# EasyVision-Ton/VMG

Hardware: AMD Instinct MI355X
Metric: LR-frames/s (train: forward+loss+backward+AdamW), VMG-REDS-few_levels 4x SR (higher is better)
Workload: dtype bf16; 1 GPU; VMG-REDS-few_levels train step, per-GPU batch 4x7x3x64x64 -> 4x SR (BASELINE configs[1]); global_batch=4, frames_per_clip=7, parallelism=dp1, launch=eager, recompute_chains=False, fp8_chains=False

## Files before the change

include/vmg_hip.h:

```cpp
#ifndef VMG_HIP_H
#define VMG_HIP_H

#include <stdint.h>

#ifdef __cplusplus
extern "C" {
#endif

#define VMG_F32 0
#define VMG_BF16 1

#define VMG_ACT_NONE 0
#define VMG_ACT_RELU 1
#define VMG_ACT_LRELU 2
#define VMG_ACT_GELU 3

#define VMG_CONV_GENERAL 0
#define VMG_CONV_KSPLIT 2
#define VMG_CONV_WS 3
#define VMG_CONV_LINEAR_WRES 4
#define VMG_CONV_WSTAT 6

const char* vmg_last_error(void);
int vmg_version(void);
// ... 36 lines not shown
  int deep;
} vmg_conv_desc;

int vmg_conv_fwd(const vmg_conv_desc* d, void* stream);
typedef struct vmg_chain_desc {
  int dtype, N, H, W, C, nblk, nsrc;
  const void* src[4];
  int64_t src_ps[4];
  int src_ch[4];
  const void* packed0;
  const float* bias0;
  float slope0;
  int cout_tiles0, deep0;
  const void* const* packed1;
  const float* const* bias1;
  const void* const* packed2;
  const float* const* bias2;
  float r_scaling;
  int cout_tiles, deep;
  void* const* y;
  void* const* t;
  void* const* g_y;
  void* const* g_t;
} vmg_chain_desc;
int vmg_resblock_chain_fwd(const vmg_chain_desc* d, void* stream);
int vmg_resblock_chain_bwd(const vmg_chain_desc* d, void* stream);

void* vmg_replay_build(void* hip_graph, int* n_ops, int* n_kernels);
int vmg_replay_kernel_info(void* replay, int idx, void** func, unsigned* grid_x, unsigned* block_x, void** first_arg);
int vmg_replay_run(void* replay, int first, int last, void* stream);
void vmg_replay_destroy(void* replay);

int vmg_pack_entry_bytes(void);
int vmg_pack_entry(void* entry, int kind, int dtype, const float* w, int O, int I, int ks, int o0, int on, int nsrc, const int* src_off,
                   const int* src_ch, int transpose_flip, int cout_tiles, void* packed, int blk0);
int vmg_pack_run(const void* plan_dev, int n, int total_blocks, void* stream);

int vmg_conv_debug_stamps(void* buf);

int vmg_conv_wgrad(int dtype, int ks, int N, int H, int W, const void* x, int64_t x_ps, int Cin, const void* dy,
                   int64_t dy_ps, int Cout, float* dW, int I_total, int o0, int i0, float* db, float scale,
                   void* stream);
int vmg_conv_wgrad_batched(int dtype, int ks, int npairs, const void* const* x, const void* const* dy, int N, int H, int W,
                           int64_t x_ps, int Cin, int64_t dy_ps, int Cout, float* dW, int I_total, int o0, int i0, float* db,
                           float scale, void* stream);

int64_t vmg_conv_wgrad_ws_bytes(void);
int vmg_conv_wgrad_batched_ws(int dtype, int ks, int npairs, const void* const* x, const void* const* dy, int N, int H, int W,
                              int64_t x_ps, int Cin, int64_t dy_ps, int Cout, float* dW, int I_total, int o0, int i0, float* db,
                              float scale, void* ws, int64_t ws_bytes, void* stream);
int vmg_conv_wgrad3_multi(int nprob, int npairs, const void* const* x, const void* const* dy, int N, int H, int W, int64_t x_ps, int Cin,
                          int64_t dy_ps, int Cout, float* const* dW, int I_total, int o0, int i0, float* const* db, const float* scales, void* ws,
                          int64_t ws_bytes, void* stream);
int vmg_conv_wgrad3_variant(int variant);
int vmg_linear_wgrad2_multi(int nprob, int npairs, const void* const* x, const void* const* dy, int64_t M, int64_t x_ps, int Cin, int64_t dy_ps,
                            int Cout, float* const* dW, int I_total, int o0, int i0, float* const* db, const float* scales, void* ws,
                            int64_t ws_bytes, void* stream);
#define VMG_WGRAD_V1 1
#define VMG_WGRAD_3 2
#define VMG_WGRAD_3B 3
#define VMG_WGRAD_L2 4
#define VMG_WGRAD_7 5
int vmg_conv_wgrad_last_kernel(void);
#define VMG_WGRAD_ENTRY_PLAIN 0
#define VMG_WGRAD_ENTRY_WS 1
#define VMG_WGRAD_ENTRY_MULTI 2
#define VMG_WGRAD_ALIGN_X16 1
#define VMG_WGRAD_ALIGN_DY16 2
#define VMG_WGRAD_ALIGN_DY2 4
#define VMG_WGRAD_PLAN_INTS 7
int vmg_conv_wgrad_plan(int entry, int dtype, int ks, int nprob, int npairs, int N, int H, int W, int64_t x_ps, int Cin, int64_t dy_ps, int Cout,
                        int I_total, int o0, int i0, int align, int64_t ws_bytes, int* plan);

int vmg_act_bwd(int dtype, const void* dy, const void* ref, void* out, int64_t n, int act, float slope, float alpha,
                void* stream);
int vmg_pixel_shuffle(int dtype, const void* in, void* out, int N, int H, int W, int c, int to_depth, void* stream);
int vmg_sum_n(int dtype, const void* const* srcs, int nsrc, void* out, int64_t n, void* stream);
int vmg_cast_clear(int dtype, float* acc, const void* add, void* out, int64_t n, void* stream);
int vmg_pair_steps(int dtype, int mode, void* const* steps, void* a, void* b, int n, int t, int64_t frame_elems, void* stream);
int vmg_frame_gather(int dtype, const void* src, void* dst, const int* idx, int64_t frame_elems, int n_src_frames, int n_dst_frames, int nsrc,
                     void* stream);
int vmg_pixel_unshuffle_actgrad(int dtype, const void* dy, const void* ref, void* out, int N, int H, int W, int c, int act, float slope,
                                float alpha, void* stream);
int vmg_layernorm_fwd(int dtype, const void* x, const float* w, const float* b, void* y, float* mean, float* rstd, int64_t M,
                      int C, float eps, void* stream);
int64_t vmg_layernorm_bwd_ws_bytes(void);
int vmg_layernorm_bwd(int dtype, int ndy, const void* const* dy, const void* x, const float* mean, const float* rstd, const float* w,
                      const void* add, void* dx, float* dw, float* db, int64_t M, int C, void* ws, void* stream);

int vmg_space_depth_ln_fwd(int dtype, int mode, const void* x, const float* w, const float* b, void* y, float* mean, float* rstd, int N, int H,
                           int W, int cseg, float eps, void* stream);
int vmg_space_depth_ln_bwd(int dtype, int mode, const void* dy, const void* x, const float* mean, const float* rstd, const float* w, void* dx,
                           float* dw, float* db, int N, int H, int W, int cseg, void* ws, void* stream);

int64_t vmg_group_reduce_ws_bytes(void);
int vmg_group_reduce(int dtype, const void* a, const void* b, const void* c3, float* out, int G, int64_t R, int C, int mode, float scale,
                     float* ws, int64_t ws_bytes, void* stream);
int vmg_group_reduce3(int dtype, const void* a, const void* b0, const void* b1, const void* b2, float* out, int G, int64_t R, int C, float scale,
                      float* ws, int64_t ws_bytes, void* stream);
int vmg_tab_elementwise(int dtype, int op, const void* p0, const void* p1, const void* p2, const float* coef, const float* add, float s,
                        void* o0, void* o1, void* o2, int64_t rows, int64_t R, int C, void* stream);

int vmg_warp_bilinear_fwd(int dtype, const void* x, const float* flow, void* out, int N, int H, int W, int C, void* stream);
int vmg_warp_bilinear_bwd(int dtype, const void* x, const float* flow, const void* dy, void* dx_acc, float* dflow, int N, int H,
                          int W, int C, void* stream);
int vmg_warp_nearest_planes(const float* loc, const float* flow, float* out, int N, int K2, int H, int W, void* stream);
// ... 157 lines not shown
```

vmg_amd/csrc/conv_wgrad.hip:

```cpp
#include <stdlib.h>
#include <algorithm>
#include <type_traits>

#include "common.h"

namespace {

constexpr int WG_MAX_PAIRS = 16;
int g_last_kernel = 0;
constexpr int last_kernel_id(int kind, int a = 0, int b = 0, int c = 0) { return kind << 24 | a << 16 | b << 8 | c; }
__device__ __attribute__((aligned(256))) unsigned int g_zero_buf[64];

__device__ __forceinline__ void glds16_hidden(const char* gsrc, char* lds_dst) {
  unsigned keep;
  const unsigned ldst = __builtin_amdgcn_readfirstlane((unsigned)(uintptr_t)LDS_PTR(lds_dst));
  asm volatile("s_mov_b32 %0, m0\n\ts_mov_b32 m0, %2\n\ts_nop 0\n\tglobal_load_lds_dwordx4 %1, off\n\ts_mov_b32 m0, %0"
               : "=&s"(keep) : "v"(gsrc), "s"(ldst) : "memory");
}

struct SlabBlock { int x, y, z; };
__device__ __forceinline__ SlabBlock xcd_slab_block(int gx, int gy, int S) {
  const int T = gx * gy * S, L = blockIdx.x;
  const int xcd = L & 7, j = L >> 3, rem = T & 7;
  const int w = xcd * (T >> 3) + (xcd < rem ? xcd : rem) + j;
// ... 518 lines not shown
#pragma unroll
    for (int jj = 0; jj < 7; ++jj) {
#ifdef VMG_DIAG
      if (!(a.dbg & 2))
#endif
      {
#pragma unroll
        for (int c = 0; c < 5; ++c) acc[c][jj] = __builtin_amdgcn_mfma_f32_16x16x32_bf16(af[c], bfg[jj], acc[c][jj], 0, 0, 0);
      }
#ifdef VMG_DIAG
      if (!(a.dbg & 4))
#endif
      bfg[jj] = tr_read(src + b_off[jj], W2_XC * 2);
    }
#ifdef VMG_DIAG
    if (!(a.dbg & 4))
#endif
    {
#pragma unroll
      for (int c = 0; c < 5; ++c) af[c] = tr_read(src + a_off + c * 32, W2_DYC * 2);
    }
    if (SYNC && h == 1) {
#ifdef VMG_DIAG
      if (!(a.dbg & 1))
#endif
      {
        if (j + 5 < nun) issue(S5);
        if (j + 6 < nun) issue(SU);
      }
    }
    return true;
  };
  for (int base = 0; base < nun; base += 6) {
    if (!unit(base + 0, std::integral_constant<int, 0>{})) break;
    if (!unit(base + 1, std::integral_constant<int, 1>{})) break;
    if (!unit(base + 2, std::integral_constant<int, 2>{})) break;
    if (!unit(base + 3, std::integral_constant<int, 3>{})) break;
    if (!unit(base + 4, std::integral_constant<int, 4>{})) break;
    if (!unit(base + 5, std::integral_constant<int, 5>{})) break;
  }
  asm volatile("s_waitcnt lgkmcnt(0)" ::: "memory");
  float* sl = a.slab + ((((long long)zz * a.gy + blk.y) * a.gx + blk.x) * W3_WAVES + wave) * (W3_TILES * 256);
#pragma unroll
  for (int c = 0; c < 5; ++c)
#pragma unroll
    for (int j = 0; j < 7; ++j) *reinterpret_cast<f32x4*>(sl + ((c * 7 + j) * 64 + lane) * 4) = acc[c][j];
  if (a.has_bias && q == 0 && blk.y == 0) {
    f32x4 pack = f32x4{0.f, 0.f, 0.f, 0.f};
    if (li < 5) pack = li == 0 ? accb[0] : (li == 1 ? accb[1] : (li == 2 ? accb[2] : (li == 3 ? accb[3] : accb[4])));
    *reinterpret_cast<f32x4*>(sl + (35 * 64 + lane) * 4) = pack;
  }
}

__global__ __launch_bounds__(W3_THREADS) void conv_wgrad3b_kernel(const Wgrad2K a) {
  extern __shared__ __attribute__((aligned(16))) char smem[];
  const int tid = threadIdx.x, lane = tid & 63;
  const int wave = __builtin_amdgcn_readfirstlane(tid >> 6);
  const int h = wave >> 2, q = wave & 3;
  SlabBlock blk = xcd_slab_block(a.gx, a.gy, a.S * a.nprob);
  const int prob = blk.z / a.S;
  const int zz = blk.z;
  blk.z -= prob * a.S;
  const char* const* xs = a.x + prob * WG_MAX_PAIRS;
  const char* const* dys = a.dy + prob * WG_MAX_PAIRS;
  const int ob = blk.x * W2_DYC, ib = blk.y * W2_XC;
  const long long u_lo = a.U * blk.z / a.S, u_hi = a.U * (blk.z + 1) / a.S;
  const char* zsrc = reinterpret_cast<const char*>(g_zero_buf);

  f32x4 acc[5][7];
#pragma unroll
  for (int c = 0; c < 5; ++c)
#pragma unroll
    for (int j = 0; j < 7; ++j) acc[c][j] = f32x4{0.f, 0.f, 0.f, 0.f};
  const bf16 one = (bf16)1.0f;
  const bf16x8 ones = {one, one, one, one, one, one, one, one};
  const bool bias_col = q == 3;

  unsigned voff[W3_SLOTS], flg[W3_SLOTS];
  const int nun = (int)(u_hi - u_lo);
  int ipair = (int)(u_lo / a.Upair), iseg, iy, in_;
  {
    const long long uu = u_lo - (long long)ipair * a.Upair;
    iseg = (int)(uu % a.SEG);
    const long long r = uu / a.SEG;
    iy = (int)(r % a.H);
    in_ = (int)(r / a.H);
  }
  const int wlast = a.W - (a.SEG - 1) * 32;
#pragma unroll
  for (int sl = 0; sl < W3_SLOTS; ++sl) {
    const int L = (sl * W3_WAVES + wave) * 64 + lane;
    if (L < W3_DYV) {
      const int pp = L / 18, v = L - pp * 18;
      voff[sl] = (unsigned)((pp * a.dy_ps + ob + v * 8) * 2);
      flg[sl] = 32u | (pp >= wlast ? 8u : 0u) | ((ob + v * 8 + 8 <= a.Cout) ? 0u : 16u);
    } else if (L < W3_VECS) {
      const int vec = L - W3_DYV, pp = vec / 6, v = vec - pp * 6;
      const int rr = pp / W2_XW, col = pp - rr * W2_XW;
      voff[sl] = (unsigned)(((long long)(rr * a.W + col) * a.x_ps + ib + v * 8) * 2);
      flg[sl] = 32u | (rr == 0 ? 1u : 0u) | (rr == 2 ? 2u : 0u) | (col == 0 ? 4u : 0u) | (col - 1 >= wlast ? 8u : 0u) | ((ib + v * 8 + 8 <= a.Cin) ? 0u : 16u);
    } else {
      voff[sl] = 0u;
      flg[sl] = 48u;
    }
  }
  const long long halo_x = (long long)(a.W + 1) * a.x_ps * 2;
  w3_u32x4 rs_dy = w3_rsrc(dys[ipair]), rs_x = w3_rsrc(xs[ipair] - halo_x);
// ... 74 lines not shown
    const char* src = smem + ((j + 1 < nun) ? SN : SU) * W3_BUF;
#ifdef VMG_DIAG
    const bool nocopy = a.dbg & 1;
#else
    constexpr bool nocopy = false;
#endif
    if (SYNC && h == 0) {
      issue(S5, j + 5 < nun && !nocopy);
      issue(SU, j + 6 < nun && !nocopy);
    }
#pragma unroll
    for (int jj = 0; jj < 7; ++jj) {
#ifdef VMG_DIAG
      if (!(a.dbg & 2))
#endif
      {
#pragma unroll
        for (int c = 0; c < 5; ++c) acc[c][jj] = __builtin_amdgcn_mfma_f32_16x16x32_bf16(af[c], bfg[jj], acc[c][jj], 0, 0, 0);
      }
#ifdef VMG_DIAG
      if (!(a.dbg & 4))
#endif
      if (jj < 6 || !bias_col) bfg[jj] = tr_read(src + b_off[jj], W2_XC * 2);
    }
#ifdef VMG_DIAG
    if (!(a.dbg & 4))
#endif
    {
#pragma unroll
      for (int c = 0; c < 5; ++c) af[c] = tr_read(src + a_off + c * 32, W2_DYC * 2);
    }
    if (SYNC && h == 1) {
      issue(S5, j + 5 < nun && !nocopy);
      issue(SU, j + 6 < nun && !nocopy);
    }
    return true;
  };
  for (int base = 0; base < nun; base += 6) {
    if (!unit(base + 0, std::integral_constant<int, 0>{})) break;
    if (!unit(base + 1, std::integral_constant<int, 1>{})) break;
    if (!unit(base + 2, std::integral_constant<int, 2>{})) break;
    if (!unit(base + 3, std::integral_constant<int, 3>{})) break;
    if (!unit(base + 4, std::integral_constant<int, 4>{})) break;
    if (!unit(base + 5, std::integral_constant<int, 5>{})) break;
  }
  asm volatile("s_waitcnt vmcnt(0)\n\ts_waitcnt lgkmcnt(0)" ::: "memory");
  float* sl = a.slab + ((((long long)zz * a.gy + blk.y) * a.gx + blk.x) * W3_WAVES + wave) * (W3_TILES * 256);
#pragma unroll
  for (int c = 0; c < 5; ++c)
#pragma unroll
    for (int j = 0; j < 7; ++j) *reinterpret_cast<f32x4*>(sl + ((c * 7 + j) * 64 + lane) * 4) = acc[c][j];
}

__global__ __launch_bounds__(256) void conv_wgrad3_reduce_kernel(const float* __restrict__ slab0, int S, int gx, int gy, int Cin, int Cout,
                                                                 const Wgrad3Out outs, int I_total, int o0, int i0, int bias_in_pad) {
  __shared__ float red[256];
  const long long per_s = (long long)gy * gx * W3_WG_FLOATS;
  const float* __restrict__ slab = slab0 + (long long)blockIdx.y * S * per_s;
  float* __restrict__ dW = outs.dW[blockIdx.y];
  float* __restrict__ db = outs.db[blockIdx.y];
  const float scale = outs.scale[blockIdx.y];
  for (long long e0 = blockIdx.x * 64LL; e0 < per_s; e0 += (long long)gridDim.x * 64) {
    const long long i = e0 + (threadIdx.x & 63);
    const float sum = slab_sum_4waves(slab, per_s, S, i, true, red);
    if (threadIdx.x >= 64) continue;
    const int r = (int)(i & 3);
    const int lane = (int)((i >> 2) & 63);
    long long qq = i >> 8;
    const int tile = (int)(qq % W3_TILES);
    qq /= W3_TILES;
    const int wave = (int)(qq % W3_WAVES);
    qq /= W3_WAVES;
    const int coblk = (int)(qq % gx), ciblk = (int)(qq / gx);
    const int h = wave >> 2, q = wave & 3;
    const int g = lane >> 4, l15 = lane & 15;
    if (tile < 35) {
      const int c = tile / 7, j = tile - c * 7;
      const int cot = h * 5 + c, col = q * 7 + j;
      if (cot < 9 && col < 27) {
        const int itile = col / 9, t = col - itile * 9;
        const int co = coblk * W2_DYC + cot * 16 + 4 * g + r;
        const int ci = ciblk * W2_XC + itile * 16 + l15;
        if (co < Cout && ci < Cin) dW[((long long)(o0 + co) * I_total + (i0 + ci)) * 9 + t] += sum * scale;
      }
    } else if (!bias_in_pad && db && q == 0 && ciblk == 0 && l15 < 5) {
      const int cot = h * 5 + l15;
      const int co = coblk * W2_DYC + cot * 16 + 4 * g + r;
      if (cot < 9 && co < Cout) db[o0 + co] += sum * scale;
    }
    if (bias_in_pad && db && tile < 35 && q == 3 && ciblk == 0 && l15 == 0 && tile % 7 == 6) {
      const int cot = h * 5 + tile / 7;
      const int co = coblk * W2_DYC + cot * 16 + 4 * g + r;
      if (cot < 9 && co < Cout) db[o0 + co] += sum * scale;
    }
  }
}

struct Lgrad2K {
  const char* x[W3_MAX_PROBS * WG_MAX_PAIRS];
  const char* dy[W3_MAX_PROBS * WG_MAX_PAIRS];
  int npairs, nprob;
  long long Mpair;
  long long Upair, U;
  long long x_ps, dy_ps;
  int Cin, Cout;
  float* slab;
  int S, has_bias;
  int gx, gy;
};
constexpr int L2_TILE_BYTES = 32 * 144 * 2;
constexpr int L2_BUF = 2 * L2_TILE_BYTES;
constexpr int L2_TILES = 10;
constexpr long long L2_WG_FLOATS = (long long)W2_WAVES * L2_TILES * 256;

__global__ __launch_bounds__(W2_THREADS, 2) void linear_wgrad2_kernel(const Lgrad2K a) {
// ... 265 lines not shown
    for (int ct = 0; ct < CT; ++ct) *reinterpret_cast<f32x4*>(sl + ((KS * KS * CT + ct) * 64 + lane) * 4) = accb[ct];
  }
}

__global__ __launch_bounds__(256) void conv_wgrad7_reduce_kernel(const float* __restrict__ slab, int S, int gx, int CT, int KS, int Cin, int Cout,
                                                                 float* __restrict__ dW, int I_total, int o0, int i0,
                                                                 float* __restrict__ db, float scale) {
  __shared__ float red[256];
  const int KK = KS * KS, wgf = (KK * CT + CT) * 256;
  const long long per_s = (long long)gx * wgf;
  for (long long e0 = blockIdx.x * 64LL; e0 < per_s; e0 += (long long)gridDim.x * 64) {
    const long long i = e0 + (threadIdx.x & 63);
    const float sum = slab_sum_4waves(slab, per_s, S, i, true, red);
    if (threadIdx.x >= 64) continue;
    const int ciblk = (int)(i / wgf);
    const int e = (int)(i - (long long)ciblk * wgf);
    const int r = e & 3, lane = (e >> 2) & 63, tile = e >> 8;
    const int g = lane >> 4, l15 = lane & 15;
    if (tile < KK * CT) {
      const int kx = tile % KS, ct = (tile / KS) % CT, ky = tile / (KS * CT);
      const int co = ct * 16 + 4 * g + r, ci = ciblk * 16 + l15;
      if (co < Cout && ci < Cin) dW[((long long)(o0 + co) * I_total + (i0 + ci)) * KK + ky * KS + kx] += sum * scale;
    } else if (db && ciblk == 0 && l15 == 0) {
      const int co = (tile - KK * CT) * 16 + 4 * g + r;
      if (co < Cout) db[o0 + co] += sum * scale;
    }
  }
}

constexpr int WG_NULL = 8;

struct WgradCall {
  int entry, dtype, ks, nprob, npairs;
  const void* const* x;
  const void* const* dy;
  int N, H, W;
  long long M;
  long long x_ps, dy_ps;
  int Cin, Cout;
  float* const* dW;
  float* const* db;
  const float* scale;
  int I_total, o0, i0;
  void* ws;
  long long ws_bytes;
};

struct WgradPlan {
  int kernel;
  int gx, gy, S;
  long long wgs;
  int slabs;
  int rblocks;
};

long long pixels(int N, int H, int W) { return N > 0 && H > 0 && W > 0 ? (long long)N * H * W : 0; }

int wgrad_pointer_facts(const WgradCall& d) {
  if (!d.x || !d.dy || !d.dW || !d.scale || (d.entry == VMG_WGRAD_ENTRY_MULTI && !d.ws)) return WG_NULL;
  if (d.nprob < 1 || d.nprob > W3_MAX_PROBS || d.npairs < 1 || d.npairs > WG_MAX_PAIRS) return 0;
  int f = VMG_WGRAD_ALIGN_X16 | VMG_WGRAD_ALIGN_DY16 | VMG_WGRAD_ALIGN_DY2;
  for (int p = 0; p < d.nprob * d.npairs; ++p) {
    if (!d.x[p] || !d.dy[p]) return WG_NULL;
    if ((uintptr_t)d.x[p] % 16) f &= ~VMG_WGRAD_ALIGN_X16;
    if ((uintptr_t)d.dy[p] % 16) f &= ~VMG_WGRAD_ALIGN_DY16;
    if ((uintptr_t)d.dy[p] % 2) f &= ~VMG_WGRAD_ALIGN_DY2;
  }
  for (int q = 0; q < d.nprob; ++q)
    if (!d.dW[q]) return WG_NULL;
  return f;
}

int wgrad_validate(const WgradCall& d, int facts) {
  const bool multi = d.entry == VMG_WGRAD_ENTRY_MULTI;
  VMG_CHECK(d.ks == 1 || d.ks == 3 || d.ks == 7, "conv_wgrad: ks must be 1, 3 or 7");
  VMG_CHECK(d.dtype == VMG_F32 || d.dtype == VMG_BF16, "conv_wgrad: bad dtype");
  VMG_CHECK(d.M > 0 && d.Cin > 0 && d.Cout > 0, "conv_wgrad: bad shape");
  VMG_CHECK(d.nprob >= 1 && d.nprob <= (multi ? W3_MAX_PROBS : 1) && d.npairs >= 1 && d.npairs <= WG_MAX_PAIRS, "conv_wgrad: 1..%d problems, 1..%d (x, dy) pairs",
            W3_MAX_PROBS, WG_MAX_PAIRS);
  VMG_CHECK(!(facts & WG_NULL), "conv_wgrad: null pointer");
  VMG_CHECK(d.x_ps >= d.Cin && d.dy_ps >= d.Cout && d.i0 >= 0 && d.i0 + d.Cin <= d.I_total && d.o0 >= 0, "conv_wgrad: bad strides / slices");
  return 0;
}

constexpr int w7_ct(int ks, int Cout) { return ks == 3 || Cout <= 16 ? 1 : Cout <= 32 ? 2 : 4; }
constexpr long long w7_wg_floats(int ks, int ct) { return (long long)(ks * ks * ct + ct) * 256; }
constexpr long long reduce_blocks(long long elems, int per_block, int most) { return (elems + per_block - 1) / per_block > most ? most : (elems + per_block - 1) / per_block; }

WgradPlan wgrad_plan(const WgradCall& d, int variant, int facts) {
  const bool multi = d.entry == VMG_WGRAD_ENTRY_MULTI, bf = d.dtype == VMG_BF16;
  const bool x16 = facts & VMG_WGRAD_ALIGN_X16, dy16 = facts & VMG_WGRAD_ALIGN_DY16, dy2 = facts & VMG_WGRAD_ALIGN_DY2;
  const bool xs8 = d.x_ps % 8 == 0, dys8 = d.dy_ps % 8 == 0;
  const long long ws_bytes = d.entry == VMG_WGRAD_ENTRY_PLAIN ? 0 : d.ws_bytes;
  const int seg = cdiv(d.W, 32);
  WgradPlan p = {};
  auto slabs = [&p](int kernel, long long S, long long groups, long long slab) {
    p.kernel = kernel; p.S = (int)S; p.wgs = groups * S; p.slabs = 1; p.rblocks = (int)reduce_blocks(slab, 64, 8192);
    return p;
  };
  if (bf && d.ks == 1 && xs8 && dys8 && d.Cin % 8 == 0 && d.Cout % 8 == 0 && x16 && dy16) {
    const long long U = cdiv64(d.M, 32) * d.npairs;
    p.gx = cdiv(d.Cout, 144); p.gy = cdiv(d.Cin, 144);
    const long long groups = (long long)p.gx * p.gy * d.nprob, slab = p.gx * p.gy * L2_WG_FLOATS;
    const long long S = std::max(1LL, std::min(512 / groups, U / 8));
    if (U >= 64 && d.nprob * S * slab * 4 <= ws_bytes) return slabs(last_kernel_id(VMG_WGRAD_L2), S, groups, slab);
  }
  if (!multi && bf && ((d.ks == 7 && d.Cout <= 64) || (d.ks == 3 && d.Cout <= 16)) && xs8 && d.Cin % 8 == 0 && x16 && dy2) {
    const long long U = (long long)d.npairs * d.N * cdiv(d.H, d.ks == 7 ? W7Geo<7>::R : W7Geo<3>::R) * seg;
    const int ct = w7_ct(d.ks, d.Cout);
    p.gx = cdiv(d.Cin, 16); p.gy = 1;
    const long long slab = p.gx * w7_wg_floats(d.ks, ct), cap = ws_bytes / (slab * 4);
    if (U < (1LL << 30) && cap >= 1) return slabs(last_kernel_id(VMG_WGRAD_7, ct, d.ks), std::max(1LL, std::min({512LL / p.gx, U / 2, cap})), p.gx, slab);
  }
  if (bf && d.ks == 3 && (multi || d.Cout > 16) && xs8 && dys8 && d.x_ps >= ((d.Cin + 7) & ~7) && d.dy_ps >= ((d.Cout + 7) & ~7) && x16 && dy16) {
    const long long U = (long long)d.N * d.H * seg * d.npairs;
    p.gx = cdiv(d.Cout, W2_DYC); p.gy = cdiv(d.Cin, W2_XC);
    const long long groups = (long long)p.gx * p.gy * d.nprob, slab = p.gx * p.gy * W3_WG_FLOATS;
    const long long S = std::max(1LL, std::min(256 / groups, U / 8));
    const long long reach = (d.M + 2LL * d.W + 40) * std::max(d.x_ps, d.dy_ps) * 2;
    if (d.nprob * S * slab * 4 <= ws_bytes) return slabs(last_kernel_id(variant == 1 && reach < (1LL << 31) ? VMG_WGRAD_3B : VMG_WGRAD_3), S, groups, slab);
  }
  if (multi) return WgradPlan{};
  const int small3 = bf && d.ks == 3 && d.Cout <= 16;
  const int ct = d.ks == 7 || small3 ? 1 : 3, it = d.ks == 1 ? 3 : small3 && d.Cin >= 64 ? 4 : 1;
  const long long U = (d.ks > 1 ? (long long)d.N * d.H * seg : cdiv64(d.M, 32)) * d.npairs;
  p.gx = cdiv(d.Cout, ct * 16); p.gy = cdiv(d.Cin, it * 16);
  const long long slab = (long long)p.gx * p.gy * (ct * 16 * it * 16 * d.ks * d.ks + ct * 16), ws_floats = ws_bytes / 4;
  long long S = std::min(1024 / ((long long)p.gx * p.gy), U / 32);
  p.slabs = d.ks == 7 && ws_bytes >= (1 << 20);
  if (p.slabs) S = std::min(S, ws_floats / slab);
  S = std::max(1LL, std::min(S, 65535LL));
  if (p.slabs && S * slab > ws_floats) p.slabs = 0;
  p.kernel = last_kernel_id(VMG_WGRAD_V1, d.ks, ct, it); p.S = (int)S; p.wgs = p.gx * p.gy * S;
  p.rblocks = p.slabs ? (int)reduce_blocks(slab, 256, 4096) : 0;
  return p;
}

template <auto Kernel>
void allow_lds(int bytes) {
  static bool done[VMG_MAX_DEVICES] = {};
  const int dev = vmg_current_device();
  if (done[dev]) return;
  (void)hipFuncSetAttribute(reinterpret_cast<const void*>(Kernel), hipFuncAttributeMaxDynamicSharedMemorySize, bytes);
  done[dev] = true;
}

template <typename T, int KS, int CT, int IT>
int launch_v1(const WgradCall& d, const WgradPlan& p, int facts, hipStream_t st) {
  using C = WgradCfg<T, KS, CT, IT>;
  static_assert(C::LDS_BYTES <= 160 * 1024, "wgrad LDS");
  WgradK k;
  memset(&k, 0, sizeof(k));
  k.vec_x = d.x_ps % C::VPL == 0 && (facts & VMG_WGRAD_ALIGN_X16);
  k.vec_dy = d.dy_ps % C::VPL == 0 && (facts & VMG_WGRAD_ALIGN_DY16);
  for (int i = 0; i < d.npairs; ++i) { k.x[i] = (const char*)d.x[i]; k.dy[i] = (const char*)d.dy[i]; }
  k.npairs = d.npairs;
  k.x_ps = d.x_ps; k.Cin = d.Cin; k.dy_ps = d.dy_ps; k.Cout = d.Cout;
  k.dW = d.dW[0]; k.I_total = d.I_total; k.o0 = d.o0; k.i0 = d.i0; k.db = d.db ? d.db[0] : nullptr; k.scale = d.scale[0];
  k.N = d.N; k.H = d.H; k.W = d.W; k.M = d.M;
  k.SEG = cdiv(d.W, 32);
  k.HB = d.H;
  k.Upair = KS > 1 ? (long long)d.N * k.HB * k.SEG : cdiv64(k.M, 32);
  k.U = k.Upair * d.npairs;
  k.S = p.S;
  k.slab = p.slabs ? (float*)d.ws : nullptr;
  allow_lds<conv_wgrad_kernel<T, KS, CT, IT>>(160 * 1024);
  hipLaunchKernelGGL((conv_wgrad_kernel<T, KS, CT, IT>), dim3(p.gx, p.gy, p.S), dim3(256), C::LDS_BYTES, st, k);
  VMG_LAUNCH_CHECK();
  if (p.slabs) {
    hipLaunchKernelGGL(wgrad_slab_reduce_kernel, dim3(p.rblocks), dim3(256), 0, st, (const float*)k.slab, k.S, p.gx, p.gy, C::DYC, C::XC, C::KK, k.Cout, k.Cin, k.dW,
                       k.I_total, k.o0, k.i0, k.db, k.scale);
    VMG_LAUNCH_CHECK();
  }
// ... 1 lines not shown
}

template <int CT, int KS>
int launch_w7(const WgradCall& d, const WgradPlan& p, int facts, hipStream_t st) {
  using C = W7Cfg<CT, KS>;
  static_assert(C::WG_FLOATS == w7_wg_floats(KS, CT), "wgrad_plan sizes the tap-row kernel's slabs");
  Wgrad7K k;
  memset(&k, 0, sizeof(k));
  for (int i = 0; i < d.npairs; ++i) { k.x[i] = (const char*)d.x[i]; k.dy[i] = (const char*)d.dy[i]; }
  k.npairs = d.npairs; k.x_ps = d.x_ps; k.dy_ps = d.dy_ps; k.Cin = d.Cin; k.Cout = d.Cout; k.slab = (float*)d.ws;
  k.vec_dy = d.dy_ps % 8 == 0 && (facts & VMG_WGRAD_ALIGN_DY16);
  k.N = d.N; k.H = d.H; k.W = d.W; k.SEG = cdiv(d.W, 32); k.HB = cdiv(d.H, W7Geo<KS>::R);
  k.Upair = d.N * k.HB * k.SEG; k.U = k.Upair * d.npairs;
  k.has_bias = d.db && d.db[0];
  k.S = p.S; k.gx = p.gx;
  allow_lds<conv_wgrad7_kernel<CT, KS>>(2 * C::BUF);
  hipLaunchKernelGGL((conv_wgrad7_kernel<CT, KS>), dim3((unsigned)p.wgs), dim3(W7Geo<KS>::THREADS), 2 * C::BUF, st, k);
  VMG_LAUNCH_CHECK();
  hipLaunchKernelGGL(conv_wgrad7_reduce_kernel, dim3(p.rblocks), dim3(256), 0, st, (const float*)k.slab, p.S, p.gx, CT, KS, k.Cin, k.Cout, d.dW[0], d.I_total, d.o0,
                     d.i0, d.db ? d.db[0] : nullptr, d.scale[0]);
  VMG_LAUNCH_CHECK();
  return 0;
}

template <typename K>
void fill_problems(K& k, Wgrad3Out& outs, const WgradCall& d, const WgradPlan& p) {
  memset(&k, 0, sizeof(k));
  memset(&outs, 0, sizeof(outs));
  for (int q = 0; q < d.nprob; ++q) {
    for (int i = 0; i < d.npairs; ++i) {
      k.x[q * WG_MAX_PAIRS + i] = (const char*)d.x[q * d.npairs + i];
      k.dy[q * WG_MAX_PAIRS + i] = (const char*)d.dy[q * d.npairs + i];
    }
    outs.dW[q] = d.dW[q];
    outs.db[q] = d.db ? d.db[q] : nullptr;
    outs.scale[q] = d.scale[q];
    k.has_bias = k.has_bias || outs.db[q] != nullptr;
  }
  k.npairs = d.npairs; k.nprob = d.nprob; k.x_ps = d.x_ps; k.dy_ps = d.dy_ps;
  k.S = p.S; k.slab = (float*)d.ws; k.gx = p.gx; k.gy = p.gy;
}

int launch_w3(const WgradCall& d, const WgradPlan& p, hipStream_t st) {
  Wgrad2K k;
  Wgrad3Out outs;
  fill_problems(k, outs, d, p);
  k.Cin = (d.Cin + 7) & ~7; k.Cout = (d.Cout + 7) & ~7;
  k.N = d.N; k.H = d.H; k.W = d.W; k.SEG = cdiv(d.W, 32);
  k.Upair = (long long)d.N * d.H * k.SEG; k.U = k.Upair * d.npairs;
#ifdef VMG_DIAG
  { const char* e = getenv("VMG_WGRAD_DBG"); k.dbg = e ? atoi(e) : 0; }
#endif
  const bool b = p.kernel == last_kernel_id(VMG_WGRAD_3B);
  if (b) {
    allow_lds<conv_wgrad3b_kernel>(160 * 1024);
    hipLaunchKernelGGL(conv_wgrad3b_kernel, dim3((unsigned)p.wgs), dim3(W3_THREADS), 6 * W3_BUF, st, k);
  } else {
    allow_lds<conv_wgrad3_kernel>(160 * 1024);
    hipLaunchKernelGGL(conv_wgrad3_kernel, dim3((unsigned)p.wgs), dim3(W3_THREADS), 6 * W3_BUF, st, k);
  }
  VMG_LAUNCH_CHECK();
  hipLaunchKernelGGL(conv_wgrad3_reduce_kernel, dim3(p.rblocks, d.nprob), dim3(256), 0, st, (const float*)d.ws, p.S, p.gx, p.gy, d.Cin, d.Cout, outs, d.I_total, d.o0, d.i0,
                     b ? 1 : 0 );
  VMG_LAUNCH_CHECK();
  return 0;
}

int launch_l2(const WgradCall& d, const WgradPlan& p, hipStream_t st) {
  Lgrad2K k;
  Wgrad3Out outs;
  fill_problems(k, outs, d, p);
  k.Cin = d.Cin; k.Cout = d.Cout;
  k.Mpair = d.M;
  k.Upair = (k.Mpair + 31) / 32; k.U = k.Upair * d.npairs;
  hipLaunchKernelGGL(linear_wgrad2_kernel, dim3((unsigned)p.wgs), dim3(W2_THREADS), 3 * L2_BUF, st, k);
  VMG_LAUNCH_CHECK();
  hipLaunchKernelGGL(linear_wgrad2_reduce_kernel, dim3(p.rblocks, d.nprob), dim3(256), 0, st, (const float*)d.ws, p.S, p.gx, p.gy, d.Cin, d.Cout, outs, d.I_total, d.o0, d.i0);
  VMG_LAUNCH_CHECK();
  return 0;
}

int wgrad_launch(const WgradCall& d, const WgradPlan& p, int facts, void* stream) {
  hipStream_t st = (hipStream_t)stream;
  g_last_kernel = p.kernel;
  const bool bf = d.dtype == VMG_BF16;
  switch (p.kernel) {
    case last_kernel_id(VMG_WGRAD_L2): return launch_l2(d, p, st);
    case last_kernel_id(VMG_WGRAD_3):
    case last_kernel_id(VMG_WGRAD_3B): return launch_w3(d, p, st);
    case last_kernel_id(VMG_WGRAD_7, 1, 3): return launch_w7<1, 3>(d, p, facts, st);
    case last_kernel_id(VMG_WGRAD_7, 1, 7): return launch_w7<1, 7>(d, p, facts, st);
    case last_kernel_id(VMG_WGRAD_7, 2, 7): return launch_w7<2, 7>(d, p, facts, st);
    case last_kernel_id(VMG_WGRAD_7, 4, 7): return launch_w7<4, 7>(d, p, facts, st);
    case last_kernel_id(VMG_WGRAD_V1, 7, 1, 1): return bf ? launch_v1<bf16, 7, 1, 1>(d, p, facts, st) : launch_v1<float, 7, 1, 1>(d, p, facts, st);
    case last_kernel_id(VMG_WGRAD_V1, 3, 1, 4): return launch_v1<bf16, 3, 1, 4>(d, p, facts, st);
    case last_kernel_id(VMG_WGRAD_V1, 3, 1, 1): return launch_v1<bf16, 3, 1, 1>(d, p, facts, st);
    case last_kernel_id(VMG_WGRAD_V1, 3, 3, 1): return bf ? launch_v1<bf16, 3, 3, 1>(d, p, facts, st) : launch_v1<float, 3, 3, 1>(d, p, facts, st);
    case last_kernel_id(VMG_WGRAD_V1, 1, 3, 3): return bf ? launch_v1<bf16, 1, 3, 3>(d, p, facts, st) : launch_v1<float, 1, 3, 3>(d, p, facts, st);
  }
  vmg_set_error("conv_wgrad: no kernel for plan %#x", p.kernel);
  return -1;
}

int g_w3_variant = 1;

int wgrad_run(const WgradCall& d, void* stream) {
  const int facts = wgrad_pointer_facts(d);
  if (wgrad_validate(d, facts)) return -1;
  const WgradPlan p = wgrad_plan(d, g_w3_variant, facts);
  VMG_CHECK(p.kernel, "conv_wgrad multi: not bf16 operands in aligned 8-channel vectors, too few pixels or too small a workspace for the large-tile kernel (use vmg_conv_wgrad_batched_ws)");
  return wgrad_launch(d, p, facts, stream);
}

}

extern "C" int vmg_conv_wgrad_last_kernel(void) { return g_last_kernel; }

extern "C" int vmg_conv_wgrad3_variant(int v) {
  const int prev = g_w3_variant;
  if (v == 0 || v == 1) g_w3_variant = v;
  return prev;
}

extern "C" int64_t vmg_conv_wgrad_ws_bytes(void) { return 320LL * W3_WG_FLOATS * 4; }

extern "C" int vmg_conv_wgrad_plan(int entry, int dtype, int ks, int nprob, int npairs, int N, int H, int W, int64_t x_ps, int Cin, int64_t dy_ps, int Cout,
                                   int I_total, int o0, int i0, int align, int64_t ws_bytes, int* plan) {
  VMG_CHECK(entry >= VMG_WGRAD_ENTRY_PLAIN && entry <= VMG_WGRAD_ENTRY_MULTI && plan, "conv_wgrad_plan: bad entry or null plan");
  const WgradCall d = {entry, dtype, ks, nprob, npairs, nullptr, nullptr, N, H, W, pixels(N, H, W), x_ps, dy_ps, Cin, Cout, nullptr, nullptr, nullptr, I_total, o0, i0,
                       nullptr, ws_bytes > 0 ? ws_bytes : 0};
  const int facts = align & (VMG_WGRAD_ALIGN_X16 | VMG_WGRAD_ALIGN_DY16 | VMG_WGRAD_ALIGN_DY2);
  if (wgrad_validate(d, facts)) return -1;
  const WgradPlan p = wgrad_plan(d, g_w3_variant, facts);
  const int out[VMG_WGRAD_PLAN_INTS] = {p.kernel, p.gx, p.gy, p.S, (int)p.wgs, p.slabs, p.rblocks};
  memcpy(plan, out, sizeof(out));
  return 0;
}

extern "C" int vmg_conv_wgrad(int dtype, int ks, int N, int H, int W, const void* x, int64_t x_ps, int Cin, const void* dy,
                              int64_t dy_ps, int Cout, float* dW, int I_total, int o0, int i0, float* db, float scale,
                              void* stream) {
  return vmg_conv_wgrad_batched(dtype, ks, 1, &x, &dy, N, H, W, x_ps, Cin, dy_ps, Cout, dW, I_total, o0, i0, db, scale, stream);
}

extern "C" int vmg_conv_wgrad_batched(int dtype, int ks, int npairs, const void* const* x, const void* const* dy, int N, int H, int W,
                                      int64_t x_ps, int Cin, int64_t dy_ps, int Cout, float* dW, int I_total, int o0, int i0,
                                      float* db, float scale, void* stream) {
  const WgradCall d = {VMG_WGRAD_ENTRY_PLAIN, dtype, ks, 1, npairs, x, dy, N, H, W, pixels(N, H, W), x_ps, dy_ps, Cin, Cout, &dW, &db, &scale, I_total, o0, i0,
                       nullptr, 0};
  return wgrad_run(d, stream);
}

extern "C" int vmg_conv_wgrad_batched_ws(int dtype, int ks, int npairs, const void* const* x, const void* const* dy, int N, int H, int W,
                                         int64_t x_ps, int Cin, int64_t dy_ps, int Cout, float* dW, int I_total, int o0, int i0,
                                         float* db, float scale, void* ws, int64_t ws_bytes, void* stream) {
  const WgradCall d = {VMG_WGRAD_ENTRY_WS, dtype, ks, 1, npairs, x, dy, N, H, W, pixels(N, H, W), x_ps, dy_ps, Cin, Cout, &dW, &db, &scale, I_total, o0, i0,
                       ws, ws && ws_bytes > 0 ? ws_bytes : 0};
  return wgrad_run(d, stream);
}

extern "C" int vmg_conv_wgrad3_multi(int nprob, int npairs, const void* const* x, const void* const* dy, int N, int H, int W, int64_t x_ps, int Cin,
                                     int64_t dy_ps, int Cout, float* const* dW, int I_total, int o0, int i0, float* const* db, const float* scales,
                                     void* ws, int64_t ws_bytes, void* stream) {
  const WgradCall d = {VMG_WGRAD_ENTRY_MULTI, VMG_BF16, 3, nprob, npairs, x, dy, N, H, W, pixels(N, H, W), x_ps, dy_ps, Cin, Cout, dW, db, scales, I_total, o0, i0,
                       ws, ws_bytes > 0 ? ws_bytes : 0};
  return wgrad_run(d, stream);
}

extern "C" int vmg_linear_wgrad2_multi(int nprob, int npairs, const void* const* x, const void* const* dy, int64_t M, int64_t x_ps, int Cin,
                                       int64_t dy_ps, int Cout, float* const* dW, int I_total, int o0, int i0, float* const* db,
                                       const float* scales, void* ws, int64_t ws_bytes, void* stream) {
  const WgradCall d = {VMG_WGRAD_ENTRY_MULTI, VMG_BF16, 1, nprob, npairs, x, dy, 0, 0, 0, M, x_ps, dy_ps, Cin, Cout, dW, db, scales, I_total, o0, i0,
                       ws, ws_bytes > 0 ? ws_bytes : 0};
// ... 3 lines not shown
```

Measured before the change: 601.8 LR-frames/s.

## Add four-wave wgrad3b kernel with larger per-wave register tiles

Adds a new 256-thread variant of the 3x3 weight-gradient MFMA kernel in which each of four waves holds 9x7 accumulator tiles instead of eight waves holding 5x7. LDS fragment reads and buffer DMA copies are interleaved into the MFMA stream, and the variant is made the default. The reduce kernel also skips empty padded tiles when bias sits in the padding. The aim is more register-level reuse and fewer LDS reads per MFMA. The cost is much higher accumulator register pressure, lower occupancy and a hand-tuned schedule.

```diff
diff --git a/include/vmg_hip.h b/include/vmg_hip.h
--- a/include/vmg_hip.h
+++ b/include/vmg_hip.h
@@ -112,6 +112,9 @@
 int vmg_conv_wgrad3_multi(int nprob, int npairs, const void* const* x, const void* const* dy, int N, int H, int W, int64_t x_ps, int Cin,
                           int64_t dy_ps, int Cout, float* const* dW, int I_total, int o0, int i0, float* const* db, const float* scales, void* ws,
                           int64_t ws_bytes, void* stream);
+#define VMG_WGRAD3_VARIANT_POINTERS 0
+#define VMG_WGRAD3_VARIANT_FOUR_WAVE 1
+#define VMG_WGRAD3_VARIANT_EIGHT_WAVE 2
 int vmg_conv_wgrad3_variant(int variant);
 int vmg_linear_wgrad2_multi(int nprob, int npairs, const void* const* x, const void* const* dy, int64_t M, int64_t x_ps, int Cin, int64_t dy_ps,
                             int Cout, float* const* dW, int I_total, int o0, int i0, float* const* db, const float* scales, void* ws,
diff --git a/vmg_amd/csrc/conv_wgrad.hip b/vmg_amd/csrc/conv_wgrad.hip
--- a/vmg_amd/csrc/conv_wgrad.hip
+++ b/vmg_amd/csrc/conv_wgrad.hip
@@ -594,7 +594,7 @@
   }
 }
 
-__global__ __launch_bounds__(W3_THREADS) void conv_wgrad3b_kernel(const Wgrad2K a) {
+__global__ __launch_bounds__(W3_THREADS) void conv_wgrad3b_kernel_w8(const Wgrad2K a) {
   extern __shared__ __attribute__((aligned(16))) char smem[];
   const int tid = threadIdx.x, lane = tid & 63;
   const int wave = __builtin_amdgcn_readfirstlane(tid >> 6);
@@ -775,6 +775,184 @@
     for (int j = 0; j < 7; ++j) *reinterpret_cast<f32x4*>(sl + ((c * 7 + j) * 64 + lane) * 4) = acc[c][j];
 }
 
+__device__ __forceinline__ void mfma_acc_tied(f32x4& acc, const bf16x8& a, const bf16x8& b) {
+  asm volatile("v_mfma_f32_16x16x32_bf16 %0, %1, %2, %0" : "+a"(acc) : "v"(a), "v"(b));
+}
+__device__ __forceinline__ void mfma_acc_settle(f32x4 (&t)[7]) {
+  asm volatile("s_nop 7\n\ts_nop 7" : "+a"(t[0]), "+a"(t[1]), "+a"(t[2]), "+a"(t[3]), "+a"(t[4]), "+a"(t[5]), "+a"(t[6]));
+}
+
+constexpr int W4_WAVES = 4, W4_THREADS = 256, W4_SLOTS = 6, W4_CT = 9;
+static_assert(W4_SLOTS * W4_WAVES == W3_SLOTS * W3_WAVES, "both bodies copy the same 24 chunks per unit");
+
+__global__ __launch_bounds__(W4_THREADS) void conv_wgrad3b_kernel(const Wgrad2K a) {
+  extern __shared__ __attribute__((aligned(16))) char smem[];
+  const int tid = threadIdx.x, lane = tid & 63;
+  const int q = __builtin_amdgcn_readfirstlane(tid >> 6);
+  SlabBlock blk = xcd_slab_block(a.gx, a.gy, a.S * a.nprob);
+  const int prob = blk.z / a.S;
+  const int zz = blk.z;
+  blk.z -= prob * a.S;
+  const char* const* xs = a.x + prob * WG_MAX_PAIRS;
+  const char* const* dys = a.dy + prob * WG_MAX_PAIRS;
+  const int ob = blk.x * W2_DYC, ib = blk.y * W2_XC;
+  const long long u_lo = a.U * blk.z / a.S, u_hi = a.U * (blk.z + 1) / a.S;
+
+  f32x4 acc[W4_CT][7];
+#pragma unroll
+  for (int c = 0; c < W4_CT; ++c)
+#pragma unroll
+    for (int j = 0; j < 7; ++j) acc[c][j] = f32x4{0.f, 0.f, 0.f, 0.f};
+  const bf16 one = (bf16)1.0f;
+  const bf16x8 ones = {one, one, one, one, one, one, one, one};
+  const bool bias_col = q == 3;
+
+  unsigned voff[W4_SLOTS], flg[W4_SLOTS];
+  const int nun = (int)(u_hi - u_lo);
+  int ipair = (int)(u_lo / a.Upair), iseg, iy, in_;
+  {
+    const long long uu = u_lo - (long long)ipair * a.Upair;
+    iseg = (int)(uu % a.SEG);
+    const long long r = uu / a.SEG;
+    iy = (int)(r % a.H);
+    in_ = (int)(r / a.H);
+  }
+  const int wlast = a.W - (a.SEG - 1) * 32;
+#pragma unroll
+  for (int sl = 0; sl < W4_SLOTS; ++sl) {
+    const int L = (sl * W4_WAVES + q) * 64 + lane;
+    if (L < W3_DYV) {
+      const int pp = L / 18, v = L - pp * 18;
+      voff[sl] = (unsigned)((pp * a.dy_ps + ob + v * 8) * 2);
+      flg[sl] = 32u | (pp >= wlast ? 8u : 0u) | ((ob + v * 8 + 8 <= a.Cout) ? 0u : 16u);
+    } else if (L < W3_VECS) {
+      const int vec = L - W3_DYV, pp = vec / 6, v = vec - pp * 6;
+      const int rr = pp / W2_XW, col = pp - rr * W2_XW;
+      voff[sl] = (unsigned)(((long long)(rr * a.W + col) * a.x_ps + ib + v * 8) * 2);
+      flg[sl] = 32u | (rr == 0 ? 1u : 0u) | (rr == 2 ? 2u : 0u) | (col == 0 ? 4u : 0u) | (col - 1 >= wlast ? 8u : 0u) | ((ib + v * 8 + 8 <= a.Cin) ? 0u : 16u);
+    } else {
+      voff[sl] = 0u;
+      flg[sl] = 48u;
+    }
+  }
+  const long long halo_x = (long long)(a.W + 1) * a.x_ps * 2;
+  w3_u32x4 rs_dy = w3_rsrc(dys[ipair]), rs_x = w3_rsrc(xs[ipair] - halo_x);
+  unsigned soff_dy, soff_x;
+  {
+    const long long row0 = ((long long)in_ * a.H + iy) * a.W + iseg * 32;
+    soff_dy = (unsigned)(row0 * a.dy_ps * 2);
+    soff_x = (unsigned)(row0 * a.x_ps * 2);
+  }
+  const unsigned a32_dy = (unsigned)(32 * a.dy_ps * 2), a32_x = (unsigned)(32 * a.x_ps * 2);
+  const unsigned arow_dy = (unsigned)(wlast * a.dy_ps * 2), arow_x = (unsigned)(wlast * a.x_ps * 2);
+  unsigned ubits = 0;
+  auto issue_slot = [&](int sl, int buf, unsigned dummy) __attribute__((always_inline)) {
+    if (sl == 0) ubits = dummy | 16u | (iy == 0 ? 1u : 0u) | (iy == a.H - 1 ? 2u : 0u) | (iseg == 0 ? 4u : 0u) | (iseg == a.SEG - 1 ? 8u : 0u);
+    static_assert(W3_DYV / 64 == 2 * W4_WAVES + 1, "chunks 0..8 of the list are dY: sl < 2, and wave 0's sl = 2");
+    const bool isdy = sl < 2 || (sl == 2 && q == 0);
+    const unsigned vo = (flg[sl] & ubits) ? 0x80000000u : voff[sl];
+    bufdma16_hidden(vo, isdy ? rs_dy : rs_x, isdy ? soff_dy : soff_x, smem + buf * W3_BUF + (sl * W4_WAVES + q) * 1024);
+  };
+  auto advance = [&]() __attribute__((always_inline)) {
+    unsigned d_dy = a32_dy, d_x = a32_x;
+    if (++iseg == a.SEG) {
+      iseg = 0;
+      d_dy = arow_dy; d_x = arow_x;
+      if (++iy == a.H) {
+        iy = 0;
+        if (++in_ == a.N) {
+          in_ = 0;
+          ++ipair;
+          if (ipair < a.npairs) {
+            rs_dy = w3_rsrc(dys[ipair]);
+            rs_x = w3_rsrc(xs[ipair] - halo_x);
+            soff_dy = 0u - d_dy;
+            soff_x = 0u - d_x;
+          }
+        }
+      }
+    }
+    soff_dy += d_dy;
+    soff_x += d_x;
+  };
+
+  const int li = lane & 15, lg = lane >> 4;
+  const int a_off = (8 * lg + (li >> 2)) * (W2_DYC * 2) + (4 * (li & 3)) * 2;
+  int b_off[7];
+#pragma unroll
+  for (int jj = 0; jj < 7; ++jj) {
+    const int col = min(q * 7 + jj, 26), itile = col / 9, tap = col - 9 * itile, ky = tap / 3, kx = tap - 3 * ky;
+    b_off[jj] = W3_DYV * 16 + ky * W2_XW * (W2_XC * 2) + (kx + 8 * lg + (li >> 2)) * (W2_XC * 2) + (itile * 16 + 4 * (li & 3)) * 2;
+  }
+
+  for (int j = 0; j < 5; ++j) {
+#pragma unroll
+    for (int sl = 0; sl < W4_SLOTS; ++sl) issue_slot(sl, j, j < nun ? 0u : 32u);
+    if (j < nun) advance();
+  }
+  asm volatile("s_waitcnt vmcnt(12)" ::: "memory");
+  __builtin_amdgcn_s_barrier();
+  asm volatile("" ::: "memory");
+  bf16x8 af[2][W4_CT], bfg[2][7];
+  if (nun > 0) {
+#pragma unroll
+    for (int c = 0; c < W4_CT; ++c) af[0][c] = tr_read(smem + a_off + c * 32, W2_DYC * 2);
+#pragma unroll
+    for (int jj = 0; jj < 7; ++jj) bfg[0][jj] = tr_read(smem + b_off[jj], W2_XC * 2);
+    if (bias_col) bfg[0][6] = ones;
+  }
+  if (bias_col) bfg[1][6] = ones;
+  auto unit = [&](int j, auto su_c) __attribute__((always_inline)) {
+    constexpr int SU = decltype(su_c)::value, SN = (SU + 1) % 6, S5 = (SU + 5) % 6;
+    constexpr bool SYNC = (SU & 1) == 0;
+    const char* src = smem + SN * W3_BUF;
+    const bool live = j + 5 < nun;
+    const unsigned dummy = live ? 0u : 32u;
+#pragma unroll
+    for (int jj = 0; jj < 7; ++jj) {
+#pragma unroll
+      for (int c = 0; c < W4_CT; ++c) {
+        mfma_acc_tied(acc[c][jj], af[SU & 1][c], bfg[SU & 1][jj]);
+        constexpr int READ0 = 9, READ_EVERY = 3;
+        const int r = jj * W4_CT + c - READ0;
+        if (r >= 0 && r % READ_EVERY == 0 && r / READ_EVERY < W4_CT + 7) {
+          const int k = r / READ_EVERY;
+          if (k < W4_CT) af[(SU + 1) & 1][k] = tr_read(src + a_off + k * 32, W2_DYC * 2);
+          else if (k - W4_CT < 6 || !bias_col) bfg[(SU + 1) & 1][k - W4_CT] = tr_read(src + b_off[k - W4_CT], W2_XC * 2);
+        }
+        constexpr int COPY0 = 11, COPY_EVERY = 7;
+        const int m = jj * W4_CT + c - COPY0;
+        if (m >= 0 && m % COPY_EVERY == 0 && m / COPY_EVERY < W4_SLOTS) issue_slot(m / COPY_EVERY, S5, dummy);
+        if (m == COPY_EVERY * (W4_SLOTS - 1) && live) advance();
+      }
+      if (SYNC && jj == 0) {
+        asm volatile("s_waitcnt vmcnt(12)" ::: "memory");
+        asm volatile("s_waitcnt lgkmcnt(0)" ::: "memory");
+        __builtin_amdgcn_s_barrier();
+        asm volatile("" ::: "memory");
+      }
+    }
+  };
+  for (int base = 0; base < nun; base += 6) {
+    unit(base + 0, std::integral_constant<int, 0>{});
+    unit(base + 1, std::integral_constant<int, 1>{});
+    unit(base + 2, std::integral_constant<int, 2>{});
+    unit(base + 3, std::integral_constant<int, 3>{});
+    unit(base + 4, std::integral_constant<int, 4>{});
+    unit(base + 5, std::integral_constant<int, 5>{});
+  }
+  asm volatile("s_waitcnt vmcnt(0)\n\ts_waitcnt lgkmcnt(0)" ::: "memory");
+  float* sl0 = a.slab + (((long long)zz * a.gy + blk.y) * a.gx + blk.x) * W3_WG_FLOATS;
+#pragma unroll
+  for (int ct = 0; ct < W4_CT; ++ct) mfma_acc_settle(acc[ct]);
+#pragma unroll
+  for (int ct = 0; ct < W4_CT; ++ct) {
+    float* sl = sl0 + ((ct / 5) * 4 + q) * (W3_TILES * 256) + ((ct % 5) * 7 * 64 + lane) * 4;
+#pragma unroll
+    for (int j = 0; j < 7; ++j) *reinterpret_cast<f32x4*>(sl + j * 256) = acc[ct][j];
+  }
+}
+
 __global__ __launch_bounds__(256) void conv_wgrad3_reduce_kernel(const float* __restrict__ slab0, int S, int gx, int gy, int Cin, int Cout,
                                                                  const Wgrad3Out outs, int I_total, int o0, int i0, int bias_in_pad) {
   __shared__ float red[256];
@@ -784,6 +962,10 @@
   float* __restrict__ db = outs.db[blockIdx.y];
   const float scale = outs.scale[blockIdx.y];
   for (long long e0 = blockIdx.x * 64LL; e0 < per_s; e0 += (long long)gridDim.x * 64) {
+    if (bias_in_pad) {
+      const long long t0 = e0 >> 8;
+      if (t0 % W3_TILES >= ((t0 / W3_TILES) % W3_WAVES >= 4 ? 28 : 35)) continue;
+    }
     const long long i = e0 + (threadIdx.x & 63);
     const float sum = slab_sum_4waves(slab, per_s, S, i, true, red);
     if (threadIdx.x >= 64) continue;
@@ -1155,6 +1337,7 @@
   long long wgs;
   int slabs;
   int rblocks;
+  int threads, lds;
 };
 
 long long pixels(int N, int H, int W) { return N > 0 && H > 0 && W > 0 ? (long long)N * H * W : 0; }
@@ -1221,7 +1404,8 @@
     const long long groups = (long long)p.gx * p.gy * d.nprob, slab = p.gx * p.gy * W3_WG_FLOATS;
     const long long S = std::max(1LL, std::min(256 / groups, U / 8));
     const long long reach = (d.M + 2LL * d.W + 40) * std::max(d.x_ps, d.dy_ps) * 2;
-    if (d.nprob * S * slab * 4 <= ws_bytes) return slabs(last_kernel_id(variant == 1 && reach < (1LL << 31) ? VMG_WGRAD_3B : VMG_WGRAD_3), S, groups, slab);
+    p.threads = variant == VMG_WGRAD3_VARIANT_FOUR_WAVE ? W4_THREADS : W3_THREADS; p.lds = 6 * W3_BUF;
+    if (d.nprob * S * slab * 4 <= ws_bytes) return slabs(last_kernel_id(variant != VMG_WGRAD3_VARIANT_POINTERS && reach < (1LL << 31) ? VMG_WGRAD_3B : VMG_WGRAD_3), S, groups, slab);
   }
   if (multi) return WgradPlan{};
   const int small3 = bf && d.ks == 3 && d.Cout <= 16;
@@ -1329,12 +1513,15 @@
   { const char* e = getenv("VMG_WGRAD_DBG"); k.dbg = e ? atoi(e) : 0; }
 #endif
   const bool b = p.kernel == last_kernel_id(VMG_WGRAD_3B);
-  if (b) {
+  if (b && p.threads == W4_THREADS) {
     allow_lds<conv_wgrad3b_kernel>(160 * 1024);
-    hipLaunchKernelGGL(conv_wgrad3b_kernel, dim3((unsigned)p.wgs), dim3(W3_THREADS), 6 * W3_BUF, st, k);
+    hipLaunchKernelGGL(conv_wgrad3b_kernel, dim3((unsigned)p.wgs), dim3(p.threads), p.lds, st, k);
+  } else if (b) {
+    allow_lds<conv_wgrad3b_kernel_w8>(160 * 1024);
+    hipLaunchKernelGGL(conv_wgrad3b_kernel_w8, dim3((unsigned)p.wgs), dim3(p.threads), p.lds, st, k);
   } else {
     allow_lds<conv_wgrad3_kernel>(160 * 1024);
-    hipLaunchKernelGGL(conv_wgrad3_kernel, dim3((unsigned)p.wgs), dim3(W3_THREADS), 6 * W3_BUF, st, k);
+    hipLaunchKernelGGL(conv_wgrad3_kernel, dim3((unsigned)p.wgs), dim3(p.threads), p.lds, st, k);
   }
   VMG_LAUNCH_CHECK();
   hipLaunchKernelGGL(conv_wgrad3_reduce_kernel, dim3(p.rblocks, d.nprob), dim3(256), 0, st, (const float*)d.ws, p.S, p.gx, p.gy, d.Cin, d.Cout, outs, d.I_total, d.o0, d.i0,
@@ -1379,7 +1566,7 @@
   return -1;
 }
 
-int g_w3_variant = 1;
+int g_w3_variant = VMG_WGRAD3_VARIANT_FOUR_WAVE;
 
 int wgrad_run(const WgradCall& d, void* stream) {
   const int facts = wgrad_pointer_facts(d);
@@ -1395,7 +1582,7 @@
 
 extern "C" int vmg_conv_wgrad3_variant(int v) {
   const int prev = g_w3_variant;
-  if (v == 0 || v == 1) g_w3_variant = v;
+  if (v >= VMG_WGRAD3_VARIANT_POINTERS && v <= VMG_WGRAD3_VARIANT_EIGHT_WAVE) g_w3_variant = v;
   return prev;
 }
 
```

Measured after the change: 600.4 LR-frames/s, median of 3. Within noise of the previous version (-0.2%).
